# mkocabas/EpipolarPose

Hardware: NVIDIA H100
Metric: multi-view samples/sec (4-view 256x256, bs32) (higher is better)
Workload: dtype f16x3 (fp32 operands split into two fp16 planes, 3-pass error-compensated wgmma f16, f32 accumulate: fp32-grade results)

## Files before the change

epipolarpose_b200/csrc/conv16.cu:

```cuda
#include "split16_common.cuh"

namespace {

constexpr int BM = 128;
constexpr int kThreads16 = 384;
constexpr int kConsumers = 256;
constexpr int kStageBudget = 200 * 1024;

struct Plan16 {
  int N, Hp, Wp;
  int Ho, Wo, Cout, os, ph, pw;
  int Wv, Hv;
  int T, CB;
  int tw, th, tn, tiles_w, tiles_h;
  int m_tiles, n_tiles;
  int accumulate;
  int m_fastest;
  int koff[EPB_MAX_TAPS];
  short dwq[EPB_MAX_TAPS], dhq[EPB_MAX_TAPS];
  unsigned char map[EPB_MAX_TAPS];
};

struct Maps16 {
  CUtensorMap a[4];
  CUtensorMap w;
};

template <int BN>
struct Cfg16 {
  static constexpr int A_PLANE = BM * 128;
  static constexpr int B_PLANE = BN * 128;
  static constexpr int A_BYTES = 2 * A_PLANE;
  static constexpr int B_BYTES = 2 * B_PLANE;
  static constexpr int STAGE = A_BYTES + B_BYTES;
  static constexpr int S_ = kStageBudget / STAGE;
  static constexpr int S = S_ > 6 ? 6 : S_;
  static constexpr int STAT_BYTES = (kConsumers / 32) * 2 * BN * 4;
  static constexpr int SMEM = S * STAGE + 1024  + 256  + STAT_BYTES;
  static_assert(SMEM <= 227 * 1024, "shared memory budget");
  static_assert(S >= 2, "ring too shallow");
};

template <int BN>
__global__ void __launch_bounds__(kThreads16, 1)
conv16_kernel(const __grid_constant__ Plan16 P, const __grid_constant__ Maps16 maps,
              const float* __restrict__ in_sc, const float* __restrict__ w_sc,
              const float* __restrict__ bias, float* __restrict__ out,
              double* __restrict__ stats) {
  using C = Cfg16<BN>;
  extern __shared__ uint8_t smem_raw[];
  const uint32_t raw = tc::smem_u32(smem_raw);
  const uint32_t base = (raw + 1023u) & ~1023u;
  uint8_t* sm = smem_raw + (base - raw);
  uint8_t* ctrl = sm + C::S * C::STAGE;
  uint64_t* bars = reinterpret_cast<uint64_t*>(ctrl);
  float* sstat = reinterpret_cast<float*>(ctrl + 256);
  const uint32_t bar0 = tc::smem_u32(bars);
  auto full_bar = [&](int s) { return bar0 + 8u * s; };
  auto empty_bar = [&](int s) { return bar0 + 8u * (8 + s); };

  const int warp = threadIdx.x >> 5, lane = threadIdx.x & 31;
  const int KB = P.T * P.CB;
  const int total_tiles = P.m_tiles * P.n_tiles;
  auto nt_of = [&](int tile) { return P.m_fastest ? tile / P.m_tiles : tile % P.n_tiles; };
  auto mt_of = [&](int tile) { return P.m_fastest ? tile % P.m_tiles : tile / P.n_tiles; };

  if (threadIdx.x == 0) {
    for (int s = 0; s < C::S; ++s) {
      tc::mbar_init(full_bar(s), 1);
      tc::mbar_init(empty_bar(s), kConsumers / 32);
    }
    tc::fence_barrier_init();
  }
  __syncthreads();

  if (warp < 4) {
    if (warp == 0 && lane == 0) {
      for (int v = 0; v < 4; ++v) tc::tma_prefetch_desc(&maps.a[v]);
      tc::tma_prefetch_desc(&maps.w);
      int stage = 0;
      uint32_t phase = 0;
      for (int tile = blockIdx.x; tile < total_tiles; tile += gridDim.x) {
        const int nt = nt_of(tile);
        int it = mt_of(tile);
        const int w0 = (it % P.tiles_w) * P.tw; it /= P.tiles_w;
        const int h0 = (it % P.tiles_h) * P.th;
        const int n0 = (it / P.tiles_h) * P.tn;
        int t = 0, cb = 0;
        for (int kb = 0; kb < KB; ++kb) {
          tc::mbar_wait(empty_bar(stage), phase ^ 1);
          const uint32_t fb = full_bar(stage);
          tc::mbar_arrive_expect_tx(fb, C::STAGE);
          const uint32_t a_dst = base + stage * C::STAGE;
          const CUtensorMap* am = &maps.a[P.map[t]];
          const int cx = cb * 64, wx = w0 + P.dwq[t], hx = h0 + P.dhq[t];
          tc::tma_load_5d(a_dst, am, fb, cx, wx, hx, n0, 0);
          tc::tma_load_5d(a_dst + C::A_PLANE, am, fb, cx, wx, hx, n0, 1);
          const uint32_t b_dst = a_dst + C::A_BYTES;
          const int kx = P.koff[t] + cx, rx = nt * BN;
          tc::tma_load_3d(b_dst, &maps.w, fb, kx, rx, 0);
          tc::tma_load_3d(b_dst + C::B_PLANE, &maps.w, fb, kx, rx, 1);
          if (++cb == P.CB) { cb = 0; ++t; }
          if (++stage == C::S) { stage = 0; phase ^= 1; }
        }
      }
    }
    return;
  }

  const int wgc = (warp >> 2) - 1;
  const int ct = threadIdx.x - 128;
  float* wstat = sstat + (ct >> 5) * 2 * BN;
  const int lr = (lane >> 2), lc = (lane & 3) * 2;
  const int ra = wgc * 64 + (warp & 3) * 16 + lr;
  const float alpha = in_sc[1] * w_sc[1];
  const int twh = P.tw * P.th;
  if (stats) {
    for (int c = ct; c < (kConsumers / 32) * 2 * BN; c += kConsumers) sstat[c] = 0.f;
    tc::named_sync(1, kConsumers);
  }
  auto flush_stats = [&](int nt) {
    tc::named_sync(1, kConsumers);
    for (int c = ct; c < 2 * BN; c += kConsumers) {
      const int which = c / BN, col = nt * BN + (c % BN);
      float v = 0.f;
#pragma unroll
      for (int w = 0; w < kConsumers / 32; ++w) {
        v += sstat[w * 2 * BN + c];
        sstat[w * 2 * BN + c] = 0.f;
      }
      if (col < P.Cout) atomicAdd(stats + (int64_t)which * P.Cout + col, (double)v);
    }
    tc::named_sync(1, kConsumers);
  };

  float acc[BN / 2];
  int stage = 0, nt_prev = -1;
  uint32_t phase = 0;
  for (int tile = blockIdx.x; tile < total_tiles; tile += gridDim.x) {
    const int nt = nt_of(tile);
    if (stats && nt_prev >= 0 && nt != nt_prev) flush_stats(nt_prev);
    nt_prev = nt;
#pragma unroll
    for (int i = 0; i < BN / 2; ++i) acc[i] = 0.f;
    int prev = -1;
    for (int kb = 0; kb < KB; ++kb) {
      tc::mbar_wait(full_bar(stage), phase);
      const uint32_t a_hi = base + stage * C::STAGE + wgc * 64 * 128;
      const uint32_t b_hi = base + stage * C::STAGE + C::A_BYTES;
      tc::fence_acc(acc);
      tc::wgmma_fence();
#pragma unroll
      for (int kk = 0; kk < 4; ++kk) {
        const uint64_t ah = tc::desc_kmajor_sw128(a_hi + kk * 32);
        const uint64_t al = tc::desc_kmajor_sw128(a_hi + C::A_PLANE + kk * 32);
        const uint64_t bh = tc::desc_kmajor_sw128(b_hi + kk * 32);
        const uint64_t bl = tc::desc_kmajor_sw128(b_hi + C::B_PLANE + kk * 32);
        tc::wgmma_f16<0, 0>(acc, al, bh, 1);
        tc::wgmma_f16<0, 0>(acc, ah, bl, 1);
        tc::wgmma_f16<0, 0>(acc, ah, bh, 1);
      }
      tc::wgmma_commit();
      tc::wgmma_wait<1>();
      tc::fence_acc(acc);
      if (prev >= 0 && lane == 0) tc::mbar_arrive(empty_bar(prev));
      prev = stage;
      if (++stage == C::S) { stage = 0; phase ^= 1; }
    }
    tc::wgmma_wait<0>();
    tc::fence_acc(acc);
    if (prev >= 0 && lane == 0) tc::mbar_arrive(empty_bar(prev));

    int it = mt_of(tile);
    const int w0 = (it % P.tiles_w) * P.tw; it /= P.tiles_w;
    const int h0 = (it % P.tiles_h) * P.th;
    const int n0 = (it / P.tiles_h) * P.tn;
    float* orow[2];
    bool srow[2];
#pragma unroll
    for (int h = 0; h < 2; ++h) {
      const int r = ra + 8 * h;
      const int w = w0 + r % P.tw, hh = h0 + (r / P.tw) % P.th, n = n0 + r / twh;
      orow[h] = (w < P.Wv && hh < P.Hv && n < P.N)
                    ? out + (((int64_t)n * P.Ho + (int64_t)hh * P.os + P.ph) * P.Wo +
                             (int64_t)w * P.os + P.pw) * P.Cout
                    : nullptr;
      srow[h] = w < P.Wp && hh < P.Hp && n < P.N;
    }
#pragma unroll
    for (int j = 0; j < BN / 8; ++j) {
      const int cl = 8 * j + lc, col = nt * BN + cl;
      float v[2][2];
      float2 b = make_float2(0.f, 0.f);
      if (bias && col < P.Cout) b = *reinterpret_cast<const float2*>(bias + col);
#pragma unroll
      for (int h = 0; h < 2; ++h) {
        v[h][0] = acc[4 * j + 2 * h] * alpha + b.x;
        v[h][1] = acc[4 * j + 2 * h + 1] * alpha + b.y;
        if (orow[h] && col < P.Cout) {
          float2* o = reinterpret_cast<float2*>(orow[h] + col);
          float2 x = make_float2(v[h][0], v[h][1]);
          if (P.accumulate) {
            const float2 pv = *o;
            x.x += pv.x; x.y += pv.y;
          }
          *o = x;
        }
      }
      if (stats) {
#pragma unroll
        for (int e = 0; e < 2; ++e) {
          const float x0 = srow[0] ? v[0][e] : 0.f, x1 = srow[1] ? v[1][e] : 0.f;
          float s1 = x0 + x1, s2 = fmaf(x0, x0, x1 * x1);
#pragma unroll
          for (int o = 4; o < 32; o <<= 1) {
            s1 += __shfl_xor_sync(0xffffffffu, s1, o);
            s2 += __shfl_xor_sync(0xffffffffu, s2, o);
          }
          if (lr == 0) {
            wstat[cl + e] += s1;
            wstat[BN + cl + e] += s2;
          }
        }
      }
    }
  }
  if (stats && nt_prev >= 0) flush_stats(nt_prev);
}

template <int BN>
int launch16(const Plan16& P, const Maps16& maps, const float* in_sc, const float* w_sc,
             const float* bias, float* out, double* stats, cudaStream_t st) {
  using C = Cfg16<BN>;
  static bool attr_set = false;
  if (!attr_set) {
    EPB_CUDA(cudaFuncSetAttribute(conv16_kernel<BN>, cudaFuncAttributeMaxDynamicSharedMemorySize,
                                  C::SMEM));
    attr_set = true;
  }
  const int64_t tiles = (int64_t)P.m_tiles * P.n_tiles;
  const int grid = (int)(tiles < kNumSMs ? tiles : kNumSMs);
  conv16_kernel<BN><<<grid, kThreads16, C::SMEM, st>>>(P, maps, in_sc, w_sc, bias, out, stats);
  EPB_LAUNCH_CHECK();
  return EPB_OK;
}

}

extern "C" __attribute__((visibility("default"))) int epb_conv16_fprop(
    const epb_conv_geom* g, const epb_half* in, const float* in_sc, const epb_half* w,
    const float* w_sc, const float* bias, float* out, double* stats, epb_stream_t stream) {
  int rc = epb_conv_geom_check(g);
  if (rc) return rc;
  EPB_CHECK_ARG(in && in_sc && w && w_sc && out);
  EPB_CHECK_ARG(g->Cin % 64 == 0 && g->Cout % 4 == 0 && g->Cout >= 4);
  EPB_CHECK_ARG(g->is == 1 || g->is == 2);
  EPB_CHECK_ARG(!(stats && g->accumulate));
  EPB_CHECK_ARG((reinterpret_cast<uintptr_t>(in) & 127) == 0 && (reinterpret_cast<uintptr_t>(w) & 15) == 0);
  EPB_CHECK_ARG((reinterpret_cast<uintptr_t>(out) & 7) == 0 && (reinterpret_cast<uintptr_t>(bias) & 7) == 0);
  Plan16 P;
  Maps16 maps;
  memset(&maps, 0, sizeof(maps));
  P.Ho = g->Ho; P.Wo = g->Wo; P.Cout = g->Cout; P.os = g->os; P.ph = g->ph; P.pw = g->pw;
  P.T = g->T; P.CB = g->Cin / 64; P.accumulate = g->accumulate;
  const bool dense = g->T == 1 && g->is == 1 && g->os == 1 && g->dh[0] == 0 && g->dw[0] == 0 &&
                     g->Hp == g->Hi && g->Wp == g->Wi && g->Hp == g->Ho && g->Wp == g->Wo;
  int N = g->N, Hi = g->Hi, Wi = g->Wi;
  P.N = g->N; P.Hp = g->Hp; P.Wp = g->Wp;
  if (dense) {
    const int64_t M = (int64_t)g->N * g->Hp * g->Wp;
    EPB_CHECK_ARG(M < (1LL << 31));
    N = 1; Hi = 1; Wi = (int)M;
    P.N = 1; P.Hp = 1; P.Wp = (int)M; P.Ho = 1; P.Wo = (int)M;
  }
  P.Wv = dense ? P.Wp : (g->Wo - g->pw + g->os - 1) / g->os;
  P.Hv = dense ? 1 : (g->Ho - g->ph + g->os - 1) / g->os;
  if (dense) { P.ph = 0; P.pw = 0; }
  epb_choose_tile(P.N, P.Hp, P.Wp, BM, P.tw, P.th, P.tn);
  P.tiles_w = (P.Wp + P.tw - 1) / P.tw;
  P.tiles_h = (P.Hp + P.th - 1) / P.th;
  const int64_t mt = (int64_t)P.tiles_w * P.tiles_h * ((P.N + P.tn - 1) / P.tn);
  EPB_CHECK_ARG(mt < (1LL << 30));
  P.m_tiles = (int)mt;
  bool need[4] = {false, false, false, false};
  for (int t = 0; t < g->T; ++t) {
    int qh, qw, dq_h, dq_w;
    epb_tap_split(g->dh[t], g->is, qh, dq_h);
    epb_tap_split(g->dw[t], g->is, qw, dq_w);
    P.map[t] = (unsigned char)(qh * 2 + qw);
    P.dhq[t] = (short)dq_h;
    P.dwq[t] = (short)dq_w;
    P.koff[t] = g->wt[t] * g->Cin;
    need[qh * 2 + qw] = true;
  }
  for (int v = 0; v < 4; ++v) {
    if (!need[v]) continue;
    rc = epb_make_act_map(&maps.a[v], in, N, Hi, Wi, g->Cin, g->is, v >> 1, v & 1, P.tw, P.th, P.tn);
    if (rc) return rc;
  }
  for (int v = 0; v < 4; ++v)
    if (!need[v]) {
      for (int u = 0; u < 4; ++u)
        if (need[u]) { maps.a[v] = maps.a[u]; break; }
    }
  P.m_fastest = stats != nullptr;
  const int bn = g->Cout <= 64 ? 64 : 128;
  P.n_tiles = (g->Cout + bn - 1) / bn;
  {
    epb_encode_tiled_fn enc = epb_get_encode_tiled();
    if (!enc) {
      epb_set_error("cuTensorMapEncodeTiled entry point unavailable");
      return EPB_ECUDA;
    }
    const int64_t K = (int64_t)g->Tw * g->Cin;
    const cuuint64_t dims[3] = {(cuuint64_t)K, (cuuint64_t)g->Cout, 2};
    const cuuint64_t strides[2] = {(cuuint64_t)K * 2, (cuuint64_t)K * 2 * g->Cout};
    const cuuint32_t box[3] = {64, (cuuint32_t)bn, 1};
    const cuuint32_t estr[3] = {1, 1, 1};
    CUresult cr = enc(&maps.w, CU_TENSOR_MAP_DATA_TYPE_FLOAT16, 3, const_cast<epb_half*>(w), dims,
                      strides, box, estr, CU_TENSOR_MAP_INTERLEAVE_NONE, CU_TENSOR_MAP_SWIZZLE_128B,
                      CU_TENSOR_MAP_L2_PROMOTION_L2_256B, CU_TENSOR_MAP_FLOAT_OOB_FILL_NONE);
    if (cr != CUDA_SUCCESS) {
      epb_set_error("cuTensorMapEncodeTiled(weights %d x %lld) failed (%d)", g->Cout, (long long)K,
                    (int)cr);
      return EPB_ECUDA;
    }
  }
  cudaStream_t st = as_stream(stream);
  if (bn == 64) return launch16<64>(P, maps, in_sc, w_sc, bias, out, stats, st);
  return launch16<128>(P, maps, in_sc, w_sc, bias, out, stats, st);
}
```

epipolarpose_b200/csrc/tc_common.cuh:

```cuda
#pragma once
#include <cuda.h>
#include <cuda_runtime.h>
#include <stdint.h>

namespace tc {

__device__ __forceinline__ uint32_t smem_u32(const void* p) {
  return (uint32_t)__cvta_generic_to_shared(p);
}

__device__ __forceinline__ void mbar_init(uint32_t bar, uint32_t count) {
  asm volatile("mbarrier.init.shared::cta.b64 [%0], %1;" ::"r"(bar), "r"(count) : "memory");
}
__device__ __forceinline__ void fence_barrier_init() {
  asm volatile("fence.mbarrier_init.release.cluster;" ::: "memory");
}
__device__ __forceinline__ void mbar_arrive(uint32_t bar) {
  asm volatile("mbarrier.arrive.shared::cta.b64 _, [%0];" ::"r"(bar) : "memory");
}
__device__ __forceinline__ void mbar_arrive_expect_tx(uint32_t bar, uint32_t bytes) {
  asm volatile("mbarrier.arrive.expect_tx.shared::cta.b64 _, [%0], %1;" ::"r"(bar), "r"(bytes)
               : "memory");
}
__device__ __forceinline__ void mbar_wait(uint32_t bar, uint32_t parity) {
  uint32_t done = 0;
  long long t0 = 0;
  while (true) {
    asm volatile(
        "{\n\t.reg .pred p;\n\t"
        "mbarrier.try_wait.parity.shared::cta.b64 p, [%1], %2, %3;\n\t"
        "selp.u32 %0, 1, 0, p;\n\t}"
        : "=r"(done)
        : "r"(bar), "r"(parity), "r"(2000u)
        : "memory");
    if (done) break;
    const long long now = clock64();
    if (t0 == 0) t0 = now;
    if (now - t0 > 4000000000LL) __trap();
  }
}

__device__ __forceinline__ void fence_proxy_async() {
  asm volatile("fence.proxy.async.shared::cta;" ::: "memory");
}

__device__ __forceinline__ void named_sync(int id, int threads) {
  asm volatile("bar.sync %0, %1;" ::"r"(id), "r"(threads) : "memory");
}

__device__ __forceinline__ void tma_prefetch_desc(const CUtensorMap* m) {
  asm volatile("prefetch.tensormap [%0];" ::"l"(m) : "memory");
}
__device__ __forceinline__ void tma_load_2d(uint32_t dst, const CUtensorMap* m, uint32_t bar,
                                            int x, int y) {
  asm volatile(
      "cp.async.bulk.tensor.2d.shared::cluster.global.mbarrier::complete_tx::bytes"
      " [%0], [%1, {%3, %4}], [%2];" ::"r"(dst), "l"(m), "r"(bar), "r"(x), "r"(y)
      : "memory");
}
__device__ __forceinline__ void tma_load_3d(uint32_t dst, const CUtensorMap* m, uint32_t bar,
                                            int c0, int c1, int c2) {
  asm volatile(
      "cp.async.bulk.tensor.3d.shared::cluster.global.mbarrier::complete_tx::bytes"
      " [%0], [%1, {%3, %4, %5}], [%2];" ::"r"(dst), "l"(m), "r"(bar), "r"(c0), "r"(c1), "r"(c2)
      : "memory");
}
__device__ __forceinline__ void tma_load_5d(uint32_t dst, const CUtensorMap* m, uint32_t bar,
                                            int c0, int c1, int c2, int c3, int c4) {
  asm volatile(
      "cp.async.bulk.tensor.5d.shared::cluster.global.mbarrier::complete_tx::bytes"
      " [%0], [%1, {%3, %4, %5, %6, %7}], [%2];" ::"r"(dst), "l"(m), "r"(bar), "r"(c0), "r"(c1),
      "r"(c2), "r"(c3), "r"(c4)
      : "memory");
}

__device__ __forceinline__ void tma_store_4d(const CUtensorMap* m, uint32_t src, int c0, int c1,
                                             int c2, int c3) {
  asm volatile(
      "cp.async.bulk.tensor.4d.global.shared::cta.tile.bulk_group [%0, {%2, %3, %4, %5}], [%1];" ::"l"(m),
      "r"(src), "r"(c0), "r"(c1), "r"(c2), "r"(c3)
      : "memory");
}
__device__ __forceinline__ void tma_reduce_add_4d(const CUtensorMap* m, uint32_t src, int c0,
                                                  int c1, int c2, int c3) {
  asm volatile(
      "cp.reduce.async.bulk.tensor.4d.global.shared::cta.add.tile.bulk_group [%0, {%2, %3, %4, %5}], [%1];" ::"l"(m),
      "r"(src), "r"(c0), "r"(c1), "r"(c2), "r"(c3)
      : "memory");
}
__device__ __forceinline__ void tma_store_commit() {
  asm volatile("cp.async.bulk.commit_group;" ::: "memory");
}
template <int N>
__device__ __forceinline__ void tma_store_wait_read() {
  asm volatile("cp.async.bulk.wait_group.read %0;" ::"n"(N) : "memory");
}
template <int N>
__device__ __forceinline__ void tma_store_wait() {
  asm volatile("cp.async.bulk.wait_group %0;" ::"n"(N) : "memory");
}
__device__ __forceinline__ void tma_load_4d(uint32_t dst, const CUtensorMap* m, uint32_t bar,
                                            int c0, int c1, int c2, int c3) {
  asm volatile(
      "cp.async.bulk.tensor.4d.shared::cluster.global.mbarrier::complete_tx::bytes"
      " [%0], [%1, {%3, %4, %5, %6}], [%2];" ::"r"(dst), "l"(m), "r"(bar), "r"(c0), "r"(c1),
      "r"(c2), "r"(c3)
      : "memory");
}

__device__ __forceinline__ void wgmma_fence() {
  asm volatile("wgmma.fence.sync.aligned;" ::: "memory");
}
__device__ __forceinline__ void wgmma_commit() {
  asm volatile("wgmma.commit_group.sync.aligned;" ::: "memory");
}
template <int N>
__device__ __forceinline__ void wgmma_wait() {
  asm volatile("wgmma.wait_group.sync.aligned %0;" ::"n"(N) : "memory");
}
template <int R>
__device__ __forceinline__ void fence_acc(float (&d)[R]) {
#pragma unroll
  for (int i = 0; i < R; ++i) asm volatile("" : "+f"(d[i])::"memory");
}

__device__ __forceinline__ uint64_t desc_kmajor_sw128(uint32_t addr) {
  return (uint64_t)((addr & 0x3FFFF) >> 4) | ((uint64_t)1 << 16) | ((uint64_t)(1024 >> 4) << 32) |
         ((uint64_t)1 << 62);
}
__device__ __forceinline__ uint64_t desc_mnmajor16_sw128(uint32_t addr, uint32_t lbo_bytes,
                                                         uint32_t sbo_bytes) {
  return (uint64_t)((addr & 0x3FFFF) >> 4) | ((uint64_t)(lbo_bytes >> 4) << 16) |
         ((uint64_t)(sbo_bytes >> 4) << 32) | ((uint64_t)1 << 62);
}

#define EPB_ACC8(i) "+f"(d[i]), "+f"(d[i + 1]), "+f"(d[i + 2]), "+f"(d[i + 3]), \
                    "+f"(d[i + 4]), "+f"(d[i + 5]), "+f"(d[i + 6]), "+f"(d[i + 7])
template <int TA, int TB>
__device__ __forceinline__ void wgmma_f16_n64(float (&d)[32], uint64_t adesc, uint64_t bdesc,
                                                int scale_d) {
  asm volatile(
      "{\n\t.reg .pred p;\n\tsetp.ne.b32 p, %34, 0;\n\t"
      "wgmma.mma_async.sync.aligned.m64n64k16.f32.f16.f16 "
      "{%0, %1, %2, %3, %4, %5, %6, %7, %8, %9, %10, %11, %12, %13, %14, %15, %16, %17,"
      "%18, %19, %20, %21, %22, %23, %24, %25, %26, %27, %28, %29, %30, %31},"
      " %32, %33, p, 1, 1, %35, %36;\n\t}"
      : EPB_ACC8(0), EPB_ACC8(8), EPB_ACC8(16), EPB_ACC8(24)
      : "l"(adesc), "l"(bdesc), "r"(scale_d), "n"(TA), "n"(TB));
}

template <int TA, int TB>
__device__ __forceinline__ void wgmma_f16_n128(float (&d)[64], uint64_t adesc, uint64_t bdesc,
                                                int scale_d) {
  asm volatile(
      "{\n\t.reg .pred p;\n\tsetp.ne.b32 p, %66, 0;\n\t"
      "wgmma.mma_async.sync.aligned.m64n128k16.f32.f16.f16 "
      "{%0, %1, %2, %3, %4, %5, %6, %7, %8, %9, %10, %11, %12, %13, %14, %15, %16, %17,"
      "%18, %19, %20, %21, %22, %23, %24, %25, %26, %27, %28, %29, %30, %31, %32, %33, %34,"
      "%35, %36, %37, %38, %39, %40, %41, %42, %43, %44, %45, %46, %47, %48, %49, %50, %51,"
      "%52, %53, %54, %55, %56, %57, %58, %59, %60, %61, %62, %63},"
      " %64, %65, p, 1, 1, %67, %68;\n\t}"
      : EPB_ACC8(0), EPB_ACC8(8), EPB_ACC8(16), EPB_ACC8(24), EPB_ACC8(32), EPB_ACC8(40), EPB_ACC8(48), EPB_ACC8(56)
      : "l"(adesc), "l"(bdesc), "r"(scale_d), "n"(TA), "n"(TB));
}

__device__ __forceinline__ void wgmma_tf32_n32(float (&d)[16], uint64_t adesc, uint64_t bdesc,
                                                 int scale_d) {
  asm volatile(
      "{\n\t.reg .pred p;\n\tsetp.ne.b32 p, %18, 0;\n\t"
      "wgmma.mma_async.sync.aligned.m64n32k8.f32.tf32.tf32 "
      "{%0, %1, %2, %3, %4, %5, %6, %7, %8, %9, %10, %11, %12, %13, %14, %15},"
      " %16, %17, p, 1, 1;\n\t}"
      : EPB_ACC8(0), EPB_ACC8(8)
      : "l"(adesc), "l"(bdesc), "r"(scale_d));
}

__device__ __forceinline__ void wgmma_tf32_n64(float (&d)[32], uint64_t adesc, uint64_t bdesc,
                                                 int scale_d) {
  asm volatile(
      "{\n\t.reg .pred p;\n\tsetp.ne.b32 p, %34, 0;\n\t"
      "wgmma.mma_async.sync.aligned.m64n64k8.f32.tf32.tf32 "
      "{%0, %1, %2, %3, %4, %5, %6, %7, %8, %9, %10, %11, %12, %13, %14, %15, %16, %17,"
      "%18, %19, %20, %21, %22, %23, %24, %25, %26, %27, %28, %29, %30, %31},"
      " %32, %33, p, 1, 1;\n\t}"
      : EPB_ACC8(0), EPB_ACC8(8), EPB_ACC8(16), EPB_ACC8(24)
      : "l"(adesc), "l"(bdesc), "r"(scale_d));
}

__device__ __forceinline__ void wgmma_tf32_n128(float (&d)[64], uint64_t adesc, uint64_t bdesc,
                                                 int scale_d) {
  asm volatile(
      "{\n\t.reg .pred p;\n\tsetp.ne.b32 p, %66, 0;\n\t"
      "wgmma.mma_async.sync.aligned.m64n128k8.f32.tf32.tf32 "
      "{%0, %1, %2, %3, %4, %5, %6, %7, %8, %9, %10, %11, %12, %13, %14, %15, %16, %17,"
      "%18, %19, %20, %21, %22, %23, %24, %25, %26, %27, %28, %29, %30, %31, %32, %33, %34,"
      "%35, %36, %37, %38, %39, %40, %41, %42, %43, %44, %45, %46, %47, %48, %49, %50, %51,"
      "%52, %53, %54, %55, %56, %57, %58, %59, %60, %61, %62, %63},"
      " %64, %65, p, 1, 1;\n\t}"
      : EPB_ACC8(0), EPB_ACC8(8), EPB_ACC8(16), EPB_ACC8(24), EPB_ACC8(32), EPB_ACC8(40), EPB_ACC8(48), EPB_ACC8(56)
      : "l"(adesc), "l"(bdesc), "r"(scale_d));
}

template <int TA, int TB>
__device__ __forceinline__ void wgmma_f16(float (&d)[32], uint64_t a, uint64_t b, int sd) {
  wgmma_f16_n64<TA, TB>(d, a, b, sd);
}
template <int TA, int TB>
__device__ __forceinline__ void wgmma_f16(float (&d)[64], uint64_t a, uint64_t b, int sd) {
  wgmma_f16_n128<TA, TB>(d, a, b, sd);
}
__device__ __forceinline__ void wgmma_tf32(float (&d)[16], uint64_t a, uint64_t b, int sd) {
  wgmma_tf32_n32(d, a, b, sd);
}
__device__ __forceinline__ void wgmma_tf32(float (&d)[32], uint64_t a, uint64_t b, int sd) {
  wgmma_tf32_n64(d, a, b, sd);
}
__device__ __forceinline__ void wgmma_tf32(float (&d)[64], uint64_t a, uint64_t b, int sd) {
  wgmma_tf32_n128(d, a, b, sd);
}

__device__ __forceinline__ float to_tf32(float x) {
  return __uint_as_float((__float_as_uint(x) + 0x1000u) & 0xffffe000u);
}
__device__ __forceinline__ float4 bn_act4(float4 x, float4 sc, float4 sh, float lb) {
  return make_float4(fmaxf(fmaf(x.x, sc.x, sh.x), lb), fmaxf(fmaf(x.y, sc.y, sh.y), lb),
                     fmaxf(fmaf(x.z, sc.z, sh.z), lb), fmaxf(fmaf(x.w, sc.w, sh.w), lb));
}

}

typedef CUresult (*epb_encode_tiled_fn)(CUtensorMap*, CUtensorMapDataType, cuuint32_t, void*,
                                        const cuuint64_t*, const cuuint64_t*, const cuuint32_t*,
                                        const cuuint32_t*, CUtensorMapInterleave, CUtensorMapSwizzle,
                                        CUtensorMapL2promotion, CUtensorMapFloatOOBfill);
epb_encode_tiled_fn epb_get_encode_tiled();
```

Baseline: 454.9.

## Add ping-pong consumer warpgroup schedule and register reallocation to split16 conv

When there are more tiles than CTAs, the two consumer warpgroups each take alternating whole 128-row tiles instead of splitting one tile by rows. They hand off the tensor cores through named barriers, so one warpgroup's epilogue (bias, store, BN stats) overlaps the other's wgmma mainloop. The producer warpgroup lowers its register budget with setmaxnreg so the consumers can hold two 64-row accumulators. This adds more barriers, a per-warpgroup stats staging area that triples the stats shared memory, and more complex stats folding, with a risk of register spills or deadlock bugs.

```diff
diff --git a/epipolarpose_b200/csrc/conv16.cu b/epipolarpose_b200/csrc/conv16.cu
--- a/epipolarpose_b200/csrc/conv16.cu
+++ b/epipolarpose_b200/csrc/conv16.cu
@@ -1,4 +1,6 @@
 #include "split16_common.cuh"
+
+#include <type_traits>
 
 namespace {
 
@@ -6,6 +8,8 @@
 constexpr int kThreads16 = 384;
 constexpr int kConsumers = 256;
 constexpr int kStageBudget = 200 * 1024;
+constexpr int kProducerRegs = 40;
+constexpr int kConsumerRegs = 232;
 
 struct Plan16 {
   int N, Hp, Wp;
@@ -16,6 +20,7 @@
   int m_tiles, n_tiles;
   int accumulate;
   int m_fastest;
+  int pingpong;
   int koff[EPB_MAX_TAPS];
   short dwq[EPB_MAX_TAPS], dhq[EPB_MAX_TAPS];
   unsigned char map[EPB_MAX_TAPS];
@@ -36,7 +41,7 @@
   static constexpr int S_ = kStageBudget / STAGE;
   static constexpr int S = S_ > 6 ? 6 : S_;
   static constexpr int STAT_BYTES = (kConsumers / 32) * 2 * BN * 4;
-  static constexpr int SMEM = S * STAGE + 1024  + 256  + STAT_BYTES;
+  static constexpr int SMEM = S * STAGE + 1024  + 256  + 3 * STAT_BYTES;
   static_assert(SMEM <= 227 * 1024, "shared memory budget");
   static_assert(S >= 2, "ring too shallow");
 };
@@ -68,13 +73,14 @@
   if (threadIdx.x == 0) {
     for (int s = 0; s < C::S; ++s) {
       tc::mbar_init(full_bar(s), 1);
-      tc::mbar_init(empty_bar(s), kConsumers / 32);
+      tc::mbar_init(empty_bar(s), P.pingpong ? 4 : kConsumers / 32);
     }
     tc::fence_barrier_init();
   }
   __syncthreads();
 
   if (warp < 4) {
+    tc::setmaxnreg_dec<kProducerRegs>();
     if (warp == 0 && lane == 0) {
       for (int v = 0; v < 4; ++v) tc::tma_prefetch_desc(&maps.a[v]);
       tc::tma_prefetch_desc(&maps.w);
@@ -108,128 +114,191 @@
     return;
   }
 
+  tc::setmaxnreg_inc<kConsumerRegs>();
   const int wgc = (warp >> 2) - 1;
-  const int ct = threadIdx.x - 128;
-  float* wstat = sstat + (ct >> 5) * 2 * BN;
+  const int wt = threadIdx.x & 127;
   const int lr = (lane >> 2), lc = (lane & 3) * 2;
-  const int ra = wgc * 64 + (warp & 3) * 16 + lr;
+  const int ra = (warp & 3) * 16 + lr;
+  const bool pp = P.pingpong;
+  const int j0 = pp ? wgc : 0, jstep = pp ? 2 : 1;
+  const uint32_t row0 = pp ? 0u : (uint32_t)wgc * 64;
+  const int n_local = total_tiles > (int)blockIdx.x
+                          ? (total_tiles - 1 - (int)blockIdx.x) / (int)gridDim.x + 1 : 0;
   const float alpha = in_sc[1] * w_sc[1];
   const int twh = P.tw * P.th;
+  const int turn_bar = 3 + wgc, other_turn_bar = 4 - wgc;
+  const int fold_bar = 5 + wgc, other_fold_bar = 6 - wgc, wg_bar = 7 + wgc;
+  const int ct = threadIdx.x - 128;
+  float* tstat = sstat + (1 + wgc) * 8 * 2 * BN;
   if (stats) {
     for (int c = ct; c < (kConsumers / 32) * 2 * BN; c += kConsumers) sstat[c] = 0.f;
     tc::named_sync(1, kConsumers);
   }
+  auto flush_col = [&](int nt, int c) {
+    const int which = c / BN, col = nt * BN + (c % BN);
+    float v = 0.f;
+#pragma unroll
+    for (int w = 0; w < kConsumers / 32; ++w) {
+      v += sstat[w * 2 * BN + c];
+      sstat[w * 2 * BN + c] = 0.f;
+    }
+    if (col < P.Cout) atomicAdd(stats + (int64_t)which * P.Cout + col, (double)v);
+  };
   auto flush_stats = [&](int nt) {
     tc::named_sync(1, kConsumers);
-    for (int c = ct; c < 2 * BN; c += kConsumers) {
-      const int which = c / BN, col = nt * BN + (c % BN);
-      float v = 0.f;
-#pragma unroll
-      for (int w = 0; w < kConsumers / 32; ++w) {
-        v += sstat[w * 2 * BN + c];
-        sstat[w * 2 * BN + c] = 0.f;
-      }
-      if (col < P.Cout) atomicAdd(stats + (int64_t)which * P.Cout + col, (double)v);
-    }
+    for (int c = ct; c < 2 * BN; c += kConsumers) flush_col(nt, c);
     tc::named_sync(1, kConsumers);
   };
 
-  float acc[BN / 2];
-  int stage = 0, nt_prev = -1;
-  uint32_t phase = 0;
-  for (int tile = blockIdx.x; tile < total_tiles; tile += gridDim.x) {
+  float acc[2][BN / 2];
+  int nt_prev = -1;
+  for (int j = j0; j < n_local; j += jstep) {
+    const int tile = blockIdx.x + j * gridDim.x;
     const int nt = nt_of(tile);
-    if (stats && nt_prev >= 0 && nt != nt_prev) flush_stats(nt_prev);
-    nt_prev = nt;
-#pragma unroll
-    for (int i = 0; i < BN / 2; ++i) acc[i] = 0.f;
-    int prev = -1;
-    for (int kb = 0; kb < KB; ++kb) {
-      tc::mbar_wait(full_bar(stage), phase);
-      const uint32_t a_hi = base + stage * C::STAGE + wgc * 64 * 128;
-      const uint32_t b_hi = base + stage * C::STAGE + C::A_BYTES;
-      tc::fence_acc(acc);
-      tc::wgmma_fence();
-#pragma unroll
-      for (int kk = 0; kk < 4; ++kk) {
-        const uint64_t ah = tc::desc_kmajor_sw128(a_hi + kk * 32);
-        const uint64_t al = tc::desc_kmajor_sw128(a_hi + C::A_PLANE + kk * 32);
-        const uint64_t bh = tc::desc_kmajor_sw128(b_hi + kk * 32);
-        const uint64_t bl = tc::desc_kmajor_sw128(b_hi + C::B_PLANE + kk * 32);
-        tc::wgmma_f16<0, 0>(acc, al, bh, 1);
-        tc::wgmma_f16<0, 0>(acc, ah, bl, 1);
-        tc::wgmma_f16<0, 0>(acc, ah, bh, 1);
+    if (stats && !pp && nt_prev >= 0 && nt != nt_prev) flush_stats(nt_prev);
+#pragma unroll
+    for (int i = 0; i < BN / 2; ++i) acc[0][i] = acc[1][i] = 0.f;
+    const uint32_t fill0 = (uint32_t)j * (uint32_t)KB;
+    int stage = (int)(fill0 % C::S);
+    uint32_t phase = (fill0 / C::S) & 1u;
+    if (pp && j > 0) tc::named_sync(turn_bar, 256);
+    auto mainloop = [&](auto nr) {
+      constexpr int NR = decltype(nr)::value;
+      int prev = -1;
+      for (int kb = 0; kb < KB; ++kb) {
+        tc::mbar_wait(full_bar(stage), phase);
+        const uint32_t a_hi = base + stage * C::STAGE + row0 * 128;
+        const uint32_t b_hi = base + stage * C::STAGE + C::A_BYTES;
+#pragma unroll
+        for (int r = 0; r < NR; ++r) tc::fence_acc(acc[r]);
+        tc::wgmma_fence();
+#pragma unroll
+        for (int kk = 0; kk < 4; ++kk) {
+          const uint64_t bh = tc::desc_kmajor_sw128(b_hi + kk * 32);
+          const uint64_t bl = tc::desc_kmajor_sw128(b_hi + C::B_PLANE + kk * 32);
+#pragma unroll
+          for (int r = 0; r < NR; ++r) {
+            const uint32_t a_r = a_hi + r * 64 * 128;
+            const uint64_t ah = tc::desc_kmajor_sw128(a_r + kk * 32);
+            const uint64_t al = tc::desc_kmajor_sw128(a_r + C::A_PLANE + kk * 32);
+            tc::wgmma_f16<0, 0>(acc[r], al, bh, 1);
+            tc::wgmma_f16<0, 0>(acc[r], ah, bl, 1);
+            tc::wgmma_f16<0, 0>(acc[r], ah, bh, 1);
+          }
+        }
+        tc::wgmma_commit();
+        tc::wgmma_wait<1>();
+#pragma unroll
+        for (int r = 0; r < NR; ++r) tc::fence_acc(acc[r]);
+        if (prev >= 0 && lane == 0) tc::mbar_arrive(empty_bar(prev));
+        prev = stage;
+        if (++stage == C::S) { stage = 0; phase ^= 1; }
       }
-      tc::wgmma_commit();
-      tc::wgmma_wait<1>();
-      tc::fence_acc(acc);
+      if (pp && j + 1 < n_local) tc::named_arrive(other_turn_bar, 256);
+      tc::wgmma_wait<0>();
+#pragma unroll
+      for (int r = 0; r < NR; ++r) tc::fence_acc(acc[r]);
       if (prev >= 0 && lane == 0) tc::mbar_arrive(empty_bar(prev));
-      prev = stage;
-      if (++stage == C::S) { stage = 0; phase ^= 1; }
-    }
-    tc::wgmma_wait<0>();
-    tc::fence_acc(acc);
-    if (prev >= 0 && lane == 0) tc::mbar_arrive(empty_bar(prev));
+    };
+    if (pp) mainloop(std::integral_constant<int, 2>{});
+    else mainloop(std::integral_constant<int, 1>{});
 
     int it = mt_of(tile);
     const int w0 = (it % P.tiles_w) * P.tw; it /= P.tiles_w;
     const int h0 = (it % P.tiles_h) * P.th;
     const int n0 = (it / P.tiles_h) * P.tn;
-    float* orow[2];
-    bool srow[2];
-#pragma unroll
-    for (int h = 0; h < 2; ++h) {
-      const int r = ra + 8 * h;
-      const int w = w0 + r % P.tw, hh = h0 + (r / P.tw) % P.th, n = n0 + r / twh;
-      orow[h] = (w < P.Wv && hh < P.Hv && n < P.N)
-                    ? out + (((int64_t)n * P.Ho + (int64_t)hh * P.os + P.ph) * P.Wo +
-                             (int64_t)w * P.os + P.pw) * P.Cout
-                    : nullptr;
-      srow[h] = w < P.Wp && hh < P.Hp && n < P.N;
-    }
-#pragma unroll
-    for (int j = 0; j < BN / 8; ++j) {
-      const int cl = 8 * j + lc, col = nt * BN + cl;
-      float v[2][2];
-      float2 b = make_float2(0.f, 0.f);
-      if (bias && col < P.Cout) b = *reinterpret_cast<const float2*>(bias + col);
+#pragma unroll
+    for (int r = 0; r < 2; ++r) {
+      if (r == 1 && !pp) break;
+      float* orow[2];
+      bool srow[2];
 #pragma unroll
       for (int h = 0; h < 2; ++h) {
-        v[h][0] = acc[4 * j + 2 * h] * alpha + b.x;
-        v[h][1] = acc[4 * j + 2 * h + 1] * alpha + b.y;
-        if (orow[h] && col < P.Cout) {
-          float2* o = reinterpret_cast<float2*>(orow[h] + col);
-          float2 x = make_float2(v[h][0], v[h][1]);
-          if (P.accumulate) {
-            const float2 pv = *o;
-            x.x += pv.x; x.y += pv.y;
+        const int rr = (int)row0 + 64 * r + ra + 8 * h;
+        const int w = w0 + rr % P.tw, hh = h0 + (rr / P.tw) % P.th, n = n0 + rr / twh;
+        orow[h] = (w < P.Wv && hh < P.Hv && n < P.N)
+                      ? out + (((int64_t)n * P.Ho + (int64_t)hh * P.os + P.ph) * P.Wo +
+                               (int64_t)w * P.os + P.pw) * P.Cout
+                      : nullptr;
+        srow[h] = w < P.Wp && hh < P.Hp && n < P.N;
+      }
+      float* sl = (pp ? tstat + r * 4 * 2 * BN : sstat + wgc * 4 * 2 * BN) + (warp & 3) * 2 * BN;
+      constexpr int G = 2;
+#pragma unroll
+      for (int jg = 0; jg < BN / 8; jg += G) {
+        float2 pv[G][2];
+#pragma unroll
+        for (int g = 0; g < G; ++g)
+#pragma unroll
+          for (int h = 0; h < 2; ++h) {
+            const int col = nt * BN + 8 * (jg + g) + lc;
+            pv[g][h] = make_float2(0.f, 0.f);
+            if (P.accumulate && orow[h] && col < P.Cout)
+              pv[g][h] = *reinterpret_cast<const float2*>(orow[h] + col);
           }
-          *o = x;
-        }
-      }
-      if (stats) {
-#pragma unroll
-        for (int e = 0; e < 2; ++e) {
-          const float x0 = srow[0] ? v[0][e] : 0.f, x1 = srow[1] ? v[1][e] : 0.f;
-          float s1 = x0 + x1, s2 = fmaf(x0, x0, x1 * x1);
-#pragma unroll
-          for (int o = 4; o < 32; o <<= 1) {
-            s1 += __shfl_xor_sync(0xffffffffu, s1, o);
-            s2 += __shfl_xor_sync(0xffffffffu, s2, o);
+#pragma unroll
+        for (int g = 0; g < G; ++g) {
+          const int jn = jg + g;
+          const int cl = 8 * jn + lc, col = nt * BN + cl;
+          float v[2][2];
+          float2 b = make_float2(0.f, 0.f);
+          if (bias && col < P.Cout) b = *reinterpret_cast<const float2*>(bias + col);
+#pragma unroll
+          for (int h = 0; h < 2; ++h) {
+            v[h][0] = acc[r][4 * jn + 2 * h] * alpha + b.x;
+            v[h][1] = acc[r][4 * jn + 2 * h + 1] * alpha + b.y;
+            if (orow[h] && col < P.Cout) {
+              float2 x = make_float2(v[h][0], v[h][1]);
+              if (P.accumulate) {
+                x.x += pv[g][h].x; x.y += pv[g][h].y;
+              }
+              *reinterpret_cast<float2*>(orow[h] + col) = x;
+            }
           }
-          if (lr == 0) {
-            wstat[cl + e] += s1;
-            wstat[BN + cl + e] += s2;
+          if (stats) {
+#pragma unroll
+            for (int e = 0; e < 2; ++e) {
+              const float x0 = srow[0] ? v[0][e] : 0.f, x1 = srow[1] ? v[1][e] : 0.f;
+              float s1 = x0 + x1, s2 = fmaf(x0, x0, x1 * x1);
+#pragma unroll
+              for (int o = 4; o < 32; o <<= 1) {
+                s1 += __shfl_xor_sync(0xffffffffu, s1, o);
+                s2 += __shfl_xor_sync(0xffffffffu, s2, o);
+              }
+              if (lr == 0) {
+                if (pp) {
+                  sl[cl + e] = s1;
+                  sl[BN + cl + e] = s2;
+                } else {
+                  sl[cl + e] += s1;
+                  sl[BN + cl + e] += s2;
+                }
+              }
+            }
           }
         }
       }
     }
-  }
-  if (stats && nt_prev >= 0) flush_stats(nt_prev);
+    if (stats && pp) {
+      tc::named_sync(wg_bar, 128);
+      if (j > 0) tc::named_sync(fold_bar, 256);
+      const int nt_before = j > 0 ? nt_of(tile - gridDim.x) : nt;
+      for (int c = wt; c < 2 * BN; c += 128) {
+        if (nt_before != nt) flush_col(nt_before, c);
+#pragma unroll
+        for (int w = 0; w < kConsumers / 32; ++w) sstat[w * 2 * BN + c] += tstat[w * 2 * BN + c];
+        if (j + 1 == n_local) flush_col(nt, c);
+      }
+      tc::named_sync(wg_bar, 128);
+      if (j + 1 < n_local) tc::named_arrive(other_fold_bar, 256);
+    }
+    nt_prev = nt;
+  }
+  if (stats && !pp && nt_prev >= 0) flush_stats(nt_prev);
 }
 
 template <int BN>
-int launch16(const Plan16& P, const Maps16& maps, const float* in_sc, const float* w_sc,
+int launch16(Plan16 P, const Maps16& maps, const float* in_sc, const float* w_sc,
              const float* bias, float* out, double* stats, cudaStream_t st) {
   using C = Cfg16<BN>;
   static bool attr_set = false;
@@ -240,6 +309,7 @@
   }
   const int64_t tiles = (int64_t)P.m_tiles * P.n_tiles;
   const int grid = (int)(tiles < kNumSMs ? tiles : kNumSMs);
+  P.pingpong = tiles > grid;
   conv16_kernel<BN><<<grid, kThreads16, C::SMEM, st>>>(P, maps, in_sc, w_sc, bias, out, stats);
   EPB_LAUNCH_CHECK();
   return EPB_OK;
diff --git a/epipolarpose_b200/csrc/tc_common.cuh b/epipolarpose_b200/csrc/tc_common.cuh
--- a/epipolarpose_b200/csrc/tc_common.cuh
+++ b/epipolarpose_b200/csrc/tc_common.cuh
@@ -47,6 +47,18 @@
 __device__ __forceinline__ void named_sync(int id, int threads) {
   asm volatile("bar.sync %0, %1;" ::"r"(id), "r"(threads) : "memory");
 }
+__device__ __forceinline__ void named_arrive(int id, int threads) {
+  asm volatile("bar.arrive %0, %1;" ::"r"(id), "r"(threads) : "memory");
+}
+
+template <int R>
+__device__ __forceinline__ void setmaxnreg_dec() {
+  asm volatile("setmaxnreg.dec.sync.aligned.u32 %0;" ::"n"(R));
+}
+template <int R>
+__device__ __forceinline__ void setmaxnreg_inc() {
+  asm volatile("setmaxnreg.inc.sync.aligned.u32 %0;" ::"n"(R));
+}
 
 __device__ __forceinline__ void tma_prefetch_desc(const CUtensorMap* m) {
   asm volatile("prefetch.tensormap [%0];" ::"l"(m) : "memory");
```

After: 467.1, median of 6. +2.7%, better.
